# zhiqiangdon/pose-adv-aug

Measured on AMD Instinct MI355X. Metric: images/sec, 2-stack HG 256x256 bs=24 per GPU, full training step, higher is better.
Workload: dtype bf16; 1 GPU; BASELINE configs[1]: 2-stack hourglass chan 256, bs=24/GPU, 256x256 MPII-shape synthetic frames (720x1280 uint8 resident in HBM), on-device HumanAug warp, heat-map MSE, RMSprop, PCKh; global_batch=24, parallelism=dp1, ranks_seen=1, devices_seen=1

## Files before the change

### include/poseadv.h

```cpp
#ifndef POSEADV_H
#define POSEADV_H
#include <stddef.h>
#include <stdint.h>
#ifdef __cplusplus
extern "C" {
#endif

const char* pa_last_error(void);
int pa_version(void);
int pa_dtype(void);
float pa_grad_scale(void);


int pa_gaussian_heatmap(const double* pts, float* out, int B, int J, int H, int W, void* stream);

int pa_weighted_l2(const float* pred, const float* gt, const float* weight, size_t n, float* loss, void* stream);
int pa_weighted_l2_grad(const float* pred, const float* gt, const float* weight, size_t n, const float* gout_dev,
                        float* dpred, void* stream);

int pa_get_preds(const float* maps, int B, int J, int H, int W, float* preds, float* maxval, void* stream);

int pa_final_preds(const float* maps, const float* center, const float* scale, const float* rot,
                   int B, int J, int H, int W, float* out, float* scratch_preds, void* stream);

// ... 176 lines not shown
int pa_hg_set_image_grad(pa_net* net, float* dimg, int layout);

int pa_hg_forward_half(pa_net* net, const float* img, const void* img4, int train);

int pa_asn_forward(pa_net* asn, pa_net* pose, int train, float* logits_scale, float* logits_rot);
const float* pa_asn_probs(const pa_net* asn);
int pa_asn_backward(pa_net* asn, pa_net* pose, const float* target_scale, const float* target_rot, float* loss);
int pa_asn_set_log_eps(pa_net* asn, float eps);

int pa_asn_forward_masks(pa_net* asn, pa_net* pose, int train, float* mask_logits);
int pa_asn_backward_masks(pa_net* asn, pa_net* pose, const float* dlogits);
int pa_hg_set_dropout_masks(pa_net* net, const float* masks);

int pa_hg_accuracy(pa_net* net, int stack, const int32_t* idxs, int nidx, float* acc, float* scratch);

int pa_hg_pckh(pa_net* net, int stack, const float* center, const float* scale, const float* rot, const float* gt_pts,
               const float* norm, const int32_t* idxs, int nidx, float* acc, float* person, float* scratch);

int pa_net_meters_async(pa_net* net, int on);

#define PA_PROF_CLASSES 12
int pa_net_profile_begin(pa_net* net);
int pa_net_profile_report(pa_net* net, double* out_host, int cap_classes, int* n_classes);
int pa_net_profile_classes(const pa_net* net, int32_t* out_host, int cap);
int pa_net_set_fin_prologue(pa_net* net, int max_rows);
int pa_net_set_pool_route(pa_net* net, int on);
int pa_net_design_bytes(const pa_net* net, double* out_host);
int pa_copy_probe(void* dst, const void* src, size_t bytes, void* stream);
int pa_copy_probe_form(void* dst, const void* src, size_t bytes, int form, void* stream);
int pa_conv2d_time(int mode, int variant, int B, int Cin, int Cout, int H, int W, int k, int iters, void* ws, float* ms_out, void* stream);
int pa_conv_plan_describe(int B, int H, int W, int Cin, int Cout, int taps, int in_mode, int add1_mode, int add2_mode, int ep_mode,
                          int ep2_mode, int fin_rows, int flags, int cus, int* out, int cap);
int pa_conv_launch_log(int* out, int cap);

int pa_net_set_multi_stream(pa_net* net, int on);

int pa_hg_debug_tensor(pa_net* net, const char* which, int grad, float* out, int* shape4);

int pa_asn_debug_tensor(pa_net* net, const char* which, int grad, float* out, int* shape4);

#ifdef __cplusplus
}
#endif
#endif
```

### pose_adv_aug_amd/_lib.py

```python
import ctypes as C
import os

import torch

_HERE = os.path.dirname(os.path.abspath(__file__))
DTYPE = os.environ.get('POSEADV_DTYPE', 'bf16').lower()
if DTYPE not in ('bf16', 'fp16'):
    raise ValueError('POSEADV_DTYPE must be bf16 or fp16')
LIB_PATH = os.path.join(_HERE, 'libposeadv_hip.so' if DTYPE == 'bf16' else 'libposeadv_hip_fp16.so')


def set_dtype(name):
    global DTYPE, LIB_PATH
    name = name.lower()
    if name not in ('bf16', 'fp16'):
        raise ValueError('dtype must be bf16 or fp16')
    if _lib is not None and name != DTYPE:
        raise PoseAdvError('the %s library is already loaded in this process' % DTYPE)
    DTYPE = name
    LIB_PATH = os.path.join(_HERE, 'libposeadv_hip.so' if name == 'bf16' else 'libposeadv_hip_fp16.so')


def act_dtype():
    return torch.bfloat16 if DTYPE == 'bf16' else torch.float16
# ... 127 lines not shown
    'pa_hg_heatmap_nhwc': (_vp, [_vp, _i]),
    'pa_hg_heatmap_nchw': (_i, [_vp, _i, _vp]),
    'pa_hg_backward': (_i, [_vp]),
    'pa_hg_backward_phase': (_i, [_vp, _i]),
    'pa_hg_bucket_range': (_i, [_vp, _i, C.POINTER(_sz), C.POINTER(_sz)]),
    'pa_hg_bucket_wait': (_i, [_vp, _i, _vp]),
    'pa_hg_train_step': (_i, [_vp, _vp, _vp, _i, _i, _vp]),
    'pa_hg_set_loss_total': (_i, [_vp, _vp]),
    'pa_hg_set_heat_grads': (_i, [_vp, C.POINTER(_vp), _i]),
    'pa_hg_set_image_grad': (_i, [_vp, _vp, _i]),
    'pa_stem_dgrad_workspace_bytes': (_sz, [_i, _i, _i]),
    'pa_stem_dgrad': (_i, [_vp, _vp, _vp, _i, _i, _i, _i, _vp, _vp]),
    'pa_hg_accuracy': (_i, [_vp, _i, _vp, _i, _vp, _vp]),
    'pa_hg_forward_half': (_i, [_vp, _vp, _vp, _i]),
    'pa_asn_forward': (_i, [_vp, _vp, _i, _vp, _vp]),
    'pa_asn_probs': (_vp, [_vp]),
    'pa_asn_backward': (_i, [_vp, _vp, _vp, _vp, _vp]),
    'pa_asn_set_log_eps': (_i, [_vp, _f]),
    'pa_hg_pckh': (_i, [_vp, _i, _vp, _vp, _vp, _vp, _vp, _vp, _i, _vp, _vp, _vp]),
    'pa_net_meters_async': (_i, [_vp, _i]),
    'pa_net_profile_begin': (_i, [_vp]),
    'pa_net_profile_report': (_i, [_vp, C.POINTER(C.c_double), _i, C.POINTER(_i)]),
    'pa_net_design_bytes': (_i, [_vp, C.POINTER(C.c_double)]),
    'pa_copy_probe': (_i, [_vp, _vp, _sz, _vp]),
    'pa_copy_probe_form': (_i, [_vp, _vp, _sz, _i, _vp]),
    'pa_params_csr': (_i, [_vp, _i, _vp, _vp]),
    'pa_net_set_fin_prologue': (_i, [_vp, _i]),
    'pa_net_set_pool_route': (_i, [_vp, _i]),
    'pa_wgrad_group_workspace_bytes': (_sz, [_vp, _i]),
    'pa_wgrad_group': (_i, [_vp, _i, _i, _vp, _vp]),
    'pa_conv2d_time': (_i, [_i] * 9 + [_vp, C.POINTER(C.c_float), _vp]),
    'pa_conv_plan_describe': (_i, [_i] * 14 + [C.POINTER(_i), _i]),
    'pa_conv_launch_log': (_i, [C.POINTER(_i), _i]),
    'pa_net_profile_classes': (_i, [_vp, C.POINTER(C.c_int32), _i]),
    'pa_net_set_multi_stream': (_i, [_vp, _i]),
    'pa_hg_debug_tensor': (_i, [_vp, C.c_char_p, _i, _vp, C.POINTER(_i)]),
    'pa_asn_debug_tensor': (_i, [_vp, C.c_char_p, _i, _vp, C.POINTER(_i)]),
}

EXPORTS = sorted(_PROTOS)


def lib():
    global _lib
    if _lib is None:
        if not os.path.isfile(LIB_PATH):
            raise PoseAdvError('%s not found: run `python -c "import __graft_entry__ as g; g.build()"` '
                               '(there is no CPU fallback)' % LIB_PATH)
        try:
            l = C.CDLL(LIB_PATH)
        except OSError as e:
            raise PoseAdvError('cannot load %s: %s' % (LIB_PATH, e))
        for name, (res, args) in _PROTOS.items():
            fn = getattr(l, name)
            fn.restype = res
            fn.argtypes = args
        if l.pa_dtype() != (0 if DTYPE == 'bf16' else 1):
            raise PoseAdvError('%s is not the %s build' % (LIB_PATH, DTYPE))
        _lib = l
    return _lib


def check(rc, what=''):
    if rc != 0:
        msg = lib().pa_last_error()
        raise PoseAdvError('%s failed (code %d): %s' % (what or 'libposeadv_hip call', rc, msg.decode() if msg else ''))
# ... 26 lines not shown
```

### pose_adv_aug_amd/csrc/conv1x1_tile.hip

```cpp
#include "common.h"
#include "kernels.h"
#include "conv_epilogue.h"
#include <stdlib.h>

PA_STAMP_DECL(pa_conv1t_clk, pa_debug_conv1t_clocks)
#ifdef PA_TUNING
#define PA_STAMPT(i) do { if ((a.dbg & 64) && blockIdx.x == (unsigned)(a.dbg >> 8) && blockIdx.y == 0 && threadIdx.x == 0) { \
        pa_conv1t_clk[2 * (i)] = __builtin_amdgcn_s_memtime(); pa_conv1t_clk[2 * (i) + 1] = wall_clock64(); } } while (0)
#else
#define PA_STAMPT(i) do { } while (0)
#endif

#ifndef PA_CONV1_UP_OCC
#define PA_CONV1_UP_OCC(up) 3
#endif
#ifndef PA_CONV1_OCC4
#define PA_CONV1_OCC4(cin, bm, bn, ld) 4
#endif
#define PA_GLOBAL_PTR(p) ((const __attribute__((address_space(1))) void*)(p))
#define PA_LDS_PTR(p) ((__attribute__((address_space(3))) void*)(p))

constexpr bool pa_conv1_occ4_inst(int CIN, int BM, int BN, int LD, bool PIN) {
    if (CIN == 128 && BM == 64 && BN == 64) return LD == PA_LD_PLAIN || PIN;
    if (CIN == 64 && BM == 128 && BN == 64) return LD == PA_LD_BNRELU;
    if (CIN == 64 && BM == 64 && BN == 128) return LD == PA_LD_PLAIN || LD == PA_LD_LIN2;
    return false;
}
constexpr int pa_conv1_occ(int CIN, int BM, int BN, int LD, int KS, bool UP, bool PIN) {
    if (pa_conv1_occ4_inst(CIN, BM, BN, LD, PIN)) return PA_CONV1_OCC4(CIN, BM, BN, LD);
    if (((CIN == 128 || KS == 32) && BM == 64) || (CIN == 64 && (BN == 64 || BM == 64))) return PA_CONV1_UP_OCC(UP);
    return 2;
}
constexpr int pa_conv1_ks(int CIN, int BM, int BN, int LD) { return (CIN == 64 && BM == 64 && BN == 128 && pa_conv1_occ(CIN, BM, BN, LD, 64, false, false) == 4) ? 32 : 64; }

template <int CIN, int BM, int BN, int LDMODE, int KS = 64, bool UP = false, int POOL = PA_POOL_EP_NONE, bool PIN = false>
__global__ __launch_bounds__(256, pa_conv1_occ(CIN, BM, BN, LDMODE, KS, UP, PIN)) void conv1x1_tile_kernel(PaConvArgs a, int nb_per_wg) {
    constexpr bool OCC4 = pa_conv1_occ(CIN, BM, BN, LDMODE, KS, UP, PIN) == 4;
    constexpr int CPP = CIN / 8;
    constexpr int NI = BN / 32, MI = BM / 32;
    constexpr int KT = CIN / KS;
    constexpr int WRI = 512 / KS;
    constexpr int NIW = (BN / 4) / WRI;
    constexpr int PSTEP = 256 / CPP;
    constexpr int NPASS = BM / PSTEP;
    constexpr bool CTAB = (BM == 64 && ((CIN == 128 && LDMODE == PA_LD_LIN2) || KS == 32)) || (CIN == 64 && (BN == 64 || BM == 64));
    __shared__ __attribute__((aligned(16))) bf16 lds[BM * CIN + 2 * BN * KS + ((CTAB || OCC4) ? 2 * BN * 8 : 0)];
    bf16* As = lds;
    bf16* wbuf = lds + BM * CIN;

    const int tid = threadIdx.x, lane = tid & 63;
    const int wave = __builtin_amdgcn_readfirstlane(tid >> 6);
    const int wm = wave & 1, wn = wave >> 1;
    const int M = a.B * a.H * a.W;
    const int m0 = blockIdx.x * BM;
    const int nb0 = blockIdx.y * nb_per_wg;
    const int nit = nb_per_wg * KT;
    PA_SET_MAIN_PRIO();
    PA_STAMPT(0);
#ifdef PA_TUNING
    if ((a.dbg >> 16) > 0 && gridDim.x > 256) {
        const int slot = ((int)blockIdx.x / 256) % 3;
        for (int i = 0; i < slot * (a.dbg >> 16); ++i) __builtin_amdgcn_s_sleep(16);
    }
#endif
// ... 138 lines not shown
            asm volatile("s_waitcnt vmcnt(0)" ::: "memory");
            __syncthreads();
        }
        if (nbi == 0) PA_STAMPT(4);
        float* T = reinterpret_cast<float*>(KS == 32 ? wbuf : wbuf + ((nbi * KT + KT - 1) & 1) * (BN * KS));
        if constexpr (UP) {
            pa_conv_epilogue_lds_up<BN, NI, MI>(a, acc, (nb0 + nbi) * BN, wm, wn, pixel_of_row,
                                                [&](int x) { return up_rp * (a.W / 2) + up_cx * (BM / 4) + (x >> 1); },
                                                T, (int)blockIdx.x, reinterpret_cast<float4*>(lds + BM * CIN + 2 * BN * KS));
        } else
        pa_conv_epilogue_auto<BN, NI, MI, (CIN == 256 || CIN == 64 || CTAB), CTAB, 256, (BN < 128), POOL, OCC4>(a, acc, (nb0 + nbi) * BN, wm, wn,
                                         [&](int wr, int mi, int p) { const int m = m0 + wr * (BM / 2) + mi * 16 + p; return m < M ? m : -1; },
                                         T, (int)blockIdx.x, (CTAB || OCC4) ? reinterpret_cast<float4*>(lds + BM * CIN + 2 * BN * KS) : nullptr);
        if (nbi == 0) PA_STAMPT(5);
        __syncthreads();
    }
    PA_STAMPT(6);
}

template <int CIN, int BM, int BN, int KS = 64, bool LIN2_ONLY = false>
static void launch_row_ld(const PaConvArgs& a, int variant, dim3 grid, int nbw, hipStream_t st) {
    if constexpr (LIN2_ONLY) {
        hipLaunchKernelGGL((conv1x1_tile_kernel<CIN, BM, BN, PA_LD_LIN2, KS>), grid, dim3(256), 0, st, a, nbw);
    } else {
        switch (variant) {
            case PA_LD_PLAIN: hipLaunchKernelGGL((conv1x1_tile_kernel<CIN, BM, BN, PA_LD_PLAIN, KS>), grid, dim3(256), 0, st, a, nbw); break;
            case PA_LD_BNRELU: hipLaunchKernelGGL((conv1x1_tile_kernel<CIN, BM, BN, PA_LD_BNRELU, KS>), grid, dim3(256), 0, st, a, nbw); break;
            default: hipLaunchKernelGGL((conv1x1_tile_kernel<CIN, BM, BN, PA_LD_LIN2, KS>), grid, dim3(256), 0, st, a, nbw); break;
        }
    }
}

int pa_launch_conv1x1_tile(const PaConvArgs& a0, const PaConvPlan& p, hipStream_t st) {
    PaConvArgs a = a0; a.dbg = pa_tuning().conv1t_dbg;
    const dim3 grid(p.gx, p.gy); const int v = p.variant(), nbw = p.nbw;
    switch (p.tiling()) {
        case PA_CT_R128_64_128_UP: hipLaunchKernelGGL((conv1x1_tile_kernel<128, 64, 128, PA_LD_LIN2, 64, true>), grid, dim3(256), 0, st, a, nbw); break;
        case PA_CT_R128_64_64_PIN: hipLaunchKernelGGL((conv1x1_tile_kernel<128, 64, 64, PA_LD_LIN2, 64, false, PA_POOL_EP_NONE, true>), grid, dim3(256), 0, st, a, nbw); break;
        case PA_CT_R256_64_128_K32: launch_row_ld<256, 64, 128, 32>(a, v, grid, nbw, st); break;
        case PA_CT_R256_64_128: launch_row_ld<256, 64, 128>(a, v, grid, nbw, st); break;
        case PA_CT_R256_64_64: launch_row_ld<256, 64, 64>(a, v, grid, nbw, st); break;
        case PA_CT_R128_64_128:
            if (v == PA_CV_POOL_BWD) hipLaunchKernelGGL((conv1x1_tile_kernel<128, 64, 128, PA_LD_LIN2, 64, false, PA_POOL_EP_BWD>), grid, dim3(256), 0, st, a, nbw);
            else if (v == PA_CV_POOL_PLAIN) hipLaunchKernelGGL((conv1x1_tile_kernel<128, 64, 128, PA_LD_LIN2, 64, false, PA_POOL_EP_PLAIN>), grid, dim3(256), 0, st, a, nbw);
            else launch_row_ld<128, 64, 128>(a, v, grid, nbw, st);
            break;
        case PA_CT_R128_64_64: launch_row_ld<128, 64, 64>(a, v, grid, nbw, st); break;
        case PA_CT_R128_128_128: launch_row_ld<128, 128, 128, 64, true>(a, v, grid, nbw, st); break;
        case PA_CT_R128_128_64: launch_row_ld<128, 128, 64, 64, true>(a, v, grid, nbw, st); break;
        case PA_CT_R64_64_128:
            switch (v) {
                case PA_LD_PLAIN: hipLaunchKernelGGL((conv1x1_tile_kernel<64, 64, 128, PA_LD_PLAIN, pa_conv1_ks(64, 64, 128, PA_LD_PLAIN)>), grid, dim3(256), 0, st, a, nbw); break;
                case PA_LD_BNRELU: hipLaunchKernelGGL((conv1x1_tile_kernel<64, 64, 128, PA_LD_BNRELU, pa_conv1_ks(64, 64, 128, PA_LD_BNRELU)>), grid, dim3(256), 0, st, a, nbw); break;
                default: hipLaunchKernelGGL((conv1x1_tile_kernel<64, 64, 128, PA_LD_LIN2, pa_conv1_ks(64, 64, 128, PA_LD_LIN2)>), grid, dim3(256), 0, st, a, nbw); break;
            }
            break;
        case PA_CT_R64_128_128: launch_row_ld<64, 128, 128>(a, v, grid, nbw, st); break;
        case PA_CT_R64_128_64: launch_row_ld<64, 128, 64>(a, v, grid, nbw, st); break;
        default: pa_set_error_msg("pa_launch_conv1x1_tile: the plan names no instance of conv1x1_tile.hip"); return 1;
    }
    return (int)hipGetLastError();
}
```

### pose_adv_aug_amd/csrc/conv_epilogue.h

```cpp
#pragma once
#include "common.h"
#include "kernels.h"
#ifndef PA_EPI_LEAN_MG
#define PA_EPI_LEAN_MG 2
#endif
#ifndef PA_EPI_STAMP
#define PA_EPI_STAMP(i) do { } while (0)
#endif

template <int BN, int NI>
__device__ __forceinline__ int pa_weight_row_of_lds_row(int lr) {
    const int wt = lr / (BN / 2), l = lr - wt * (BN / 2);
    const int ni = l >> 4, rr = l & 15;
    return wt * (BN / 2) + 32 * (ni >> 1) + 8 * (rr >> 2) + 4 * (ni & 1) + (rr & 3);
}

template <int BN, int NI>
__device__ __forceinline__ int pa_lds_row_of_weight_row(int c) {
    const int wt = c / (BN / 2), l = c - wt * (BN / 2);
    const int ch = l >> 5, rem = l & 31;
    const int q = rem >> 3, h = (rem >> 2) & 1, j = rem & 3;
    return wt * (BN / 2) + (2 * ch + h) * 16 + 4 * q + j;
}

// ... 319 lines not shown
            } else {
                if constexpr (POOL) {
                    PaPoolRaw r;
                    pa_pool_request(a.add2, (unsigned)m, (unsigned)a.W, (unsigned)N, (unsigned)n, idx, r);
                    pa_read8(a.add1, idx, n, e1);
#pragma unroll
                    for (int j = 0; j < 8; ++j) e2[j] = pa_pool_value(r, pool_e, j);
                } else {
                pa_read8(a.add1, idx, n, e1);
                pa_read8(a.add2, idx, n, e2);
                }
            }
            bf16x8 o;
#pragma unroll
            for (int j = 0; j < 8; ++j) {
                float v = (j < 4 ? v0[j & 3] : v1[j & 3]) + bias[j] + e1[j] + e2[j];
                o[j] = (bf16)v;
                float rv = (float)o[j];
                s1[j] += rv;
                s2[j] += rv * rv;
            }
            *reinterpret_cast<bf16x8*>(a.out + idx) = o;
        }
        PA_EPI_STAMP(8 + 2 * mi);
    }
    if (a.ep.mode != PA_OUT_PLAIN) {
        PA_EPI_STAMP(11);
        pa_lds_barrier();
        const f32x2 v = pa_stats_reduce<BN, NT, TSMALL>(s1, s2, T);
        if (tid < BN) *reinterpret_cast<f32x2*>(a.ep.stats + ((size_t)stat_row * N + n0 + tid) * 2) = v;
    }
}

template <int BN, int NI, int MI, bool TAB, int NT = 256, bool TSMALL = false, bool FUSE = false, bool POOL = false, bool LEAN = false, class PixFn>
__device__ __forceinline__ void pa_conv_epilogue_lds_bwd(const PaConvArgs& a, f32x4 (&acc)[NI][MI], int n0, int wm, int wn,
                                                         PixFn pix, float* T, int stat_row, float4* ctab = nullptr) {
    constexpr int CPR = BN / 8;
    constexpr int RPS = NT / CPR;
    constexpr int SW = (NT / 8) / RPS;
    constexpr int NW = NT / 64;
    constexpr int G = FUSE ? MI : ((MI >= 2 && !TAB) ? 2 : 1);
    constexpr int ROWS = NT / 8;
    static_assert(!FUSE || !TAB, "fused staging: constants in registers");
    constexpr int IT = G * SW;
    int tid = threadIdx.x;
    if constexpr (LEAN) asm volatile("" : "+v"(tid));
    const int lane = tid & 63;
    const int N = a.Cout;
    const int chunk = tid % CPR, rsub = tid / CPR;
    const int n = n0 + chunk * 8;
    const int m1 = a.add1.mode, m2 = a.add2.mode;
    float s1[8], s2[8], es[8], et[8], ka[8], kb[8], kc[8];
#pragma unroll
    for (int j = 0; j < 8; ++j) { s1[j] = 0.f; s2[j] = 0.f; }
    const int wrow = wm * 16 + (lane & 15);
    const int wslot0 = (wn * (BN / 2)) / 4 + 2 * (lane >> 4);
#pragma unroll
    for (int g = 0; g < MI; g += G) {
        unsigned idx[IT];
        bool ok[IT];
        bf16x8 xr[IT], p1[IT], q1[IT], p2[POOL ? 1 : IT];
        PaPoolRaw pr[POOL ? IT : 1];
        const bool pool_e = POOL && a.add2.q != nullptr;
#pragma unroll
        for (int pp = 0; pp < G; ++pp)
#pragma unroll
            for (int sw = 0; sw < SW; ++sw) {
                const int it = pp * SW + sw, r = sw * RPS + rsub;
                const int m = pix(r >> 4, g + pp, r & 15);
                ok[it] = m >= 0;
                idx[it] = ok[it] ? (unsigned)m * (unsigned)N + (unsigned)n : 0u;
#ifdef PA_TUNING
                if (a.dbg & 16) { xr[it] = bf16x8{}; p1[it] = bf16x8{}; q1[it] = bf16x8{}; p2[it] = bf16x8{}; continue; }
#endif
// ... 119 lines not shown
                r0[j] = (float)o0[j]; r1[j] = (float)o1[j];
            }
            *reinterpret_cast<bf16x8*>(a.out + i0) = o0;
            *reinterpret_cast<bf16x8*>(a.out + i1) = o1;
        }
        bf16x8 ol;
#pragma unroll
        for (int j = 0; j < 8; ++j) {
            const float q0 = __shfl_xor(r0[j], 16, 64), q1 = __shfl_xor(r1[j], 16, 64);
            const float sum = ((r0[j] + q0) + r1[j]) + q1;
            const float4 e = ctab[j * CPR + chunk];
            const float xv = (float)xl[j];
            const float dz = (fmaf(e.x, xv, e.y) > 0.f) ? sum : 0.f;
            ol[j] = (bf16)dz;
            if (!(rsub & 1)) { const float dzr = (float)ol[j]; l1[j] += dzr; l2[j] += dzr * xv; }
        }
        if (!(rsub & 1)) *reinterpret_cast<bf16x8*>(a.out2 + il) = ol;
    }
    float cm = 0.f, ci = 0.f;
    if (tid < BN) { cm = a.ep2.mean[n0 + tid]; ci = a.ep2.invstd[n0 + tid]; }
    pa_lds_barrier();
    const f32x2 t = pa_stats_reduce<BN, NT, false>(l1, l2, T);
    if (tid < BN) {
        f32x2 v = {t[0], ci * (t[1] - cm * t[0])};
        *reinterpret_cast<f32x2*>(a.ep2.stats + ((size_t)stat_row * N + n0 + tid) * 2) = v;
    }
}

__host__ __device__ inline bool pa_bwd_epilogue_lds_ok(const PaConvArgs& a) {
    return a.xcd < 2 && a.bias == nullptr && (a.add1.mode == PA_LD_NONE || a.add1.mode == PA_LD_PLAIN || a.add1.mode == PA_LD_LIN2) &&
           (a.add2.mode == PA_LD_NONE || a.add2.mode == PA_LD_PLAIN);
}

template <int BN, int NI, int MI, bool BWD_LDS = true, bool TAB = false, int NT = 256, bool TSMALL = false, int POOL = 0, bool LEAN = false, class PixFn>
__device__ __forceinline__ void pa_conv_epilogue_auto(const PaConvArgs& a, f32x4 (&acc)[NI][MI], int n0, int wm, int wn,
                                                      PixFn pix, float* T, int stat_row, float4* ctab = nullptr) {
    constexpr bool FUSE = !TSMALL && !TAB && MI > 1 && MI * BN <= 128;
    if constexpr (POOL == PA_POOL_EP_BWD) {
        pa_conv_epilogue_lds_bwd<BN, NI, MI, TAB, NT, TSMALL, FUSE, true>(a, acc, n0, wm, wn, pix, T, stat_row, ctab);
        return;
    } else if constexpr (POOL == PA_POOL_EP_PLAIN) {
        pa_conv_epilogue_lds<BN, NI, MI, NT, TSMALL, FUSE, true>(a, acc, n0, wm, wn, pix, T, stat_row);
        return;
    }
    if (a.ep.mode == PA_OUT_BWD) {
        const bool lds_ok = BWD_LDS && pa_bwd_epilogue_lds_ok(a);
        if (lds_ok) {
            pa_conv_epilogue_lds_bwd<BN, NI, MI, (TAB || LEAN), NT, TSMALL, FUSE, false, LEAN>(a, acc, n0, wm, wn, pix, T, stat_row, ctab);
        } else if constexpr (TAB || NT != 256) {
            __builtin_trap();
        } else {
            const int p = threadIdx.x & 15;
            pa_conv_epilogue<BN, NI, MI, (LEAN && MI > PA_EPI_LEAN_MG) ? PA_EPI_LEAN_MG : MI>(a, acc, n0, wm, wn, [&](int mi) { return pix(wm, mi, p); }, T, stat_row);
        }
    } else {
        pa_conv_epilogue_lds<BN, NI, MI, NT, TSMALL, FUSE, false, LEAN>(a, acc, n0, wm, wn, pix, T, stat_row, ctab);
    }
}
```

### pose_adv_aug_amd/csrc/kernels.h

```cpp
#pragma once
#include "common.h"
#include "bn_fin.h"
#include "launch_plan.h"
#include "wgrad_plan.h"
#include "conv_plan.h"

struct PaConvArgs {
    PaOperand in;
    const bf16* w;
    const float* bias;
    PaOperand add1;
    PaOperand add2;
    PaEpilogue ep;
    bf16* out;
    int B, H, W, Cin, Cout, taps;
    bf16* dz_out;
    PaBnFin fin;
    int low_prio;
    int dbg;
    int xcd;
    PaEpilogue ep2;
    bf16* out2;
};
int pa_conv_cus();
inline PaConvShape pa_conv_shape(const PaConvArgs& a) {
    return PaConvShape{a.B, a.H, a.W, a.Cin, a.Cout, a.taps, a.in.mode, a.add1.mode, a.add2.mode, a.ep.mode, a.ep2.mode, a.fin.rows, a.bias != nullptr,
                       a.out2 != nullptr, a.dz_out != nullptr, a.in.map != nullptr, a.in.q != nullptr, a.ep2.scale && a.ep2.shift, a.add2.map != nullptr,
                       pa_conv_cus()};
}
int pa_launch_conv(const PaConvArgs& a, const PaConvPlan& p, hipStream_t st, int* stat_rows = nullptr);
inline int pa_launch_conv(const PaConvArgs& a, hipStream_t st, int* stat_rows = nullptr) { return pa_launch_conv(a, pa_conv_plan(pa_conv_shape(a)), st, stat_rows); }
int pa_launch_conv3x3_tile(const PaConvArgs& a, const PaConvPlan& p, hipStream_t st);
int pa_launch_conv1x1_tile(const PaConvArgs& a, const PaConvPlan& p, hipStream_t st);
inline int pa_max_stat_rows(int M) { int r = (M + 63) / 64; return r < 512 ? 512 : r; }

struct PaWgradArgs {
    PaOperand dy;
    PaOperand x;
    float* part;
    float* dbpart;
    int B, H, W, Cin, Cout, taps, splits;
};
int pa_launch_wgrad(const PaWgradArgs& a, hipStream_t st);
int pa_launch_stem_wgrad_tile(const PaWgradArgs& a, const PaWgradPlan& p, hipStream_t st);
int pa_launch_wgrad_tile(const PaWgradArgs& a, const PaWgradPlan& p, hipStream_t st);
int pa_wgrad_job_workgroups(const PaWgradArgs& a);
struct PaWgradReduceJob;
int pa_launch_wgrad_group(const PaWgradArgs* const* jobs, int n, hipStream_t st, bool keep_order = false,
                          const PaWgradReduceJob* red_jobs = nullptr, const int* red_idx = nullptr, int red_n = 0);
void pa_wgrad_set_launch_flags(unsigned flags);

struct PaWgradReduceJob {
    const float* part; float* dst; const float* dbpart; float* dbdst;
    int Cout, Cin, taps, splits, real_cout, real_cin;
};
int pa_launch_wgrad_reduce(const PaWgradReduceJob* jobs_dev, int njobs, int max_elems, hipStream_t st);
#define PA_RED_LIST_MAX 24
struct PaRedList { int idx[PA_RED_LIST_MAX]; };
int pa_launch_wgrad_reduce_list(const PaWgradReduceJob* jobs_dev, const int* idx, int n, int max_elems, hipStream_t st);

int pa_launch_bn_fin(const PaBnFin& f, int C, hipStream_t st);
int pa_launch_bn_fin2(const PaBnFin& a, int Ca, const PaBnFin& b, int Cb, hipStream_t st);
struct PaBnEvalJob { const float* gamma; const float* beta; const float* rmean; const float* rvar; float* scale; float* shift; int C; };
int pa_launch_bn_eval(const PaBnEvalJob* jobs_dev, int njobs, float eps, hipStream_t st);

int pa_launch_maxpool_fwd(const PaOperand& in, bf16* out, int B, int H, int W, int C, hipStream_t st, unsigned char* map = nullptr, bf16* xmax = nullptr);
// ... 63 lines not shown
```

### pose_adv_aug_amd/csrc/tuning.h

```cpp
#pragma once
#include <stdlib.h>

#define PA_TUNING_TABLE(X)                                                                                                           \
                                                                      \
    X(conv1_old,        "PA_CONV1_OLD",        0,   "1x1 convolutions on the generic kernel (no row-tile kernel, no fused upsample-add gradient)") \
    X(conv3_old,        "PA_CONV3_OLD",        0,   "3x3 convolutions on the generic kernel (no halo-tile kernel)")                 \
    X(wgrad_old,        "PA_WGRAD_OLD",        0,   "weight gradients on the generic kernel (no tile kernel, stem included)")       \
    X(stem_wgrad_old,   "PA_STEM_WGRAD_OLD",   0,   "the stem's weight gradient on the generic kernel")                            \
    X(eltwise_old,      "PA_ELTWISE_OLD",      0,   "pooling / upsample-add / cell-mask launches in their first, unvectorised form") \
    X(conv3_nosmall,    "PA_CONV3_NOSMALL",    0,   "no 8 x 8 / 4 x 4 halo tiles: the small maps go to the generic kernel")        \
    X(igemm_oneshot,    "PA_IGEMM_ONESHOT",    1,   "0: the small 1x1 layers on the K-stepping generic kernel instead of the one-shot one") \
    X(no_dz3,           "PA_NO_DZ3",           0,   "conv3's data gradient does not store dz3 (its readers recompute it)")         \
    X(no_dz2,           "PA_NO_DZ2",           0,   "conv2's data gradient does not store dz2")                                    \
    X(epi_bwd_direct,   "PA_EPI_BWD_DIRECT",   0,   "direct (no LDS) BatchNorm-backward epilogue wherever an instance carries both") \
    X(conv3_noxcd,      "PA_CONV3_NOXCD",      0,   "3x3 tiles in launch order instead of one contiguous range per XCD")           \
    X(wg_group,         "PA_WG_GROUP",         1,   "0: one launch per weight gradient instead of group launches")                 \
    X(wg_red_in_group,  "PA_WG_RED_IN_GROUP",  1,   "0: slab reductions as launches of their own instead of inside the next group launch") \
    X(wgrad_anyorder,   "PA_WGRAD_ANYORDER",   1,   "0: ungrouped weight gradients of one flush as ordinary in-order launches")    \
    X(wgrad_nopipe,     "PA_WGRAD_NOPIPE",     0,   "plain instead of pipelined tile weight gradients")                            \
    X(upadd_fuse,       "PA_UPADD_FUSE",       1,   "0: the upsample-add backward's low-resolution half as a launch of its own")   \
    X(upadd_split,      "PA_UPADD_SPLIT",      1,   "0: both halves of the upsample-add backward in one launch on the main stream") \
    X(pool_route,       "PA_POOL_ROUTE",       3,   "pool gradients through the forward pools' arg-max maps: bit 0 the hourglass pools, bit 1 the stem's pool (0: a pool backward launch each)") \
    X(fin_prologue,     "PA_FIN_PROLOGUE",     128, "most partial rows a consumer finalizes in its prologue (0: always a finalize launch; at most 128)") \
    X(fin_mask,         "PA_FIN_MASK",         7,   "which finalizes may ride in a consumer: 1 forward x1 / x2, 2 backward x2, 4 backward x3") \
    X(single_stream,    "PA_SINGLE_STREAM",    0,   "everything on the caller's stream")                                           \
    X(no_wstream,       "PA_NO_WSTREAM",       0,   "side streams, but the weight gradients on the stream that produced their operands") \
    X(stem_on_main,     "PA_STEM_ON_MAIN",     1,   "0: the stem's weight gradient on the weight-gradient stream")                 \
                                                              \
    X(wgrad_wgs1,       "PA_WGRAD_WGS1",       256, "workgroup target of a 1x1 tile weight gradient launched alone")               \
    X(wgrad_wgs9,       "PA_WGRAD_WGS9",       256, "the same for 3x3")                                                            \
    X(wgrad_min1,       "PA_WGRAD_MIN1",       3,   "fewest 128-pixel tiles for which a 1x1 weight gradient takes the tile kernel") \
    X(wg_group_wgs1,    "PA_WG_GROUP_WGS1",    64,  "workgroup budget of a 1x1 job of a group launch")                             \
    X(wg_group_wgs9,    "PA_WG_GROUP_WGS9",    64,  "the same for 3x3")                                                            \
    X(wg_group_minper1, "PA_WG_GROUP_MINPER1", 2,   "fewest tiles per workgroup of a 1x1 job")                                     \
    X(wg_group_minper9, "PA_WG_GROUP_MINPER9", 4,   "the same for 3x3")                                                            \
    X(wg_group_cap,     "PA_WG_GROUP_CAP",     256, "most workgroups of one group launch")                                         \
    X(wg_red_wgs,       "PA_WG_RED_WGS",       256, "workgroups of the slab reduction inside a group launch")                      \
    X(wreduce_lag,      "PA_WREDUCE_LAG",      2,   "flushes whose slabs wait in the stash before they are summed")                \
    X(stem_splits,      "PA_STEM_SPLITS",      512, "splits (slabs) of the stem's weight gradient")                                \
    X(wgrad_tile1,      "PA_WGRAD_TILE1",      0,   "generic 1x1 weight gradient: forced tile variant (0: by shape)")              \
    X(wgrad_tile9,      "PA_WGRAD_TILE9",      0,   "the same for 3x3")                                                            \
    X(wgrad_blocks,     "PA_WGRAD_BLOCKS",     0,   "generic weight gradient: forced split count (0: by shape)")                   \
                                                                                    \
    X(ablate,           "PA_ABLATE",           0,   "INSTRUMENT, wrong results: mask of launch classes that are skipped (net.hip)") \
    X(ablate_h,         "PA_ABLATE_H",         8,   "INSTRUMENT: largest map height the low-resolution bits of PA_ABLATE skip")    \
    X(conv3_dbg,        "PA_CONV3_DBG",        0,   "INSTRUMENT, wrong results: phase ablation / tap rotation / cycle stamps of the 3x3 tile kernel") \
    X(conv1_dbg,        "PA_CONV1_DBG",        0,   "INSTRUMENT, timing only: cycle stamps of the one-shot 1x1 kernel")            \
    X(conv1t_dbg,       "PA_CONV1T_DBG",       0,   "INSTRUMENT, timing only: cycle stamps of the row-tile 1x1 kernel")            \
    X(fin_anyorder,     "PA_FIN_ANYORDER",     0,   "INSTRUMENT, results may be wrong: finalize launches without ordering behind their producer")

struct PaTuning {
#define PA_TUNING_FIELD(field, env, value, doc) int field = value;
    PA_TUNING_TABLE(PA_TUNING_FIELD)
#undef PA_TUNING_FIELD
};

#ifdef PA_TUNING
inline const PaTuning& pa_tuning() {
    static const PaTuning t = [] {
        PaTuning v;
#define PA_TUNING_READ(field, env, value, doc) if (const char* e = getenv(env)) v.field = atoi(e);
        PA_TUNING_TABLE(PA_TUNING_READ)
#undef PA_TUNING_READ
        return v;
    }();
    return t;
}
#else
inline const PaTuning& pa_tuning() {
    static constexpr PaTuning t{};
    return t;
}
// ... 2 lines not shown
```

Baseline: 4296 images/sec.

## Add persistent multi-tile 1x1 conv kernel that keeps weights resident in LDS

Result: no change. 4313 images/sec (median of 4 runs) (+0.4%).

```diff
diff --git a/include/poseadv.h b/include/poseadv.h
--- a/include/poseadv.h
+++ b/include/poseadv.h
@@ -232,6 +232,8 @@
 int pa_conv_plan_describe(int B, int H, int W, int Cin, int Cout, int taps, int in_mode, int add1_mode, int add2_mode, int ep_mode,
                           int ep2_mode, int fin_rows, int flags, int cus, int* out, int cap);
 int pa_conv_launch_log(int* out, int cap);
+int pa_conv1_stream_set(int mode);
+int pa_conv1_stream_launches(long long* out, int cap);
 
 int pa_net_set_multi_stream(pa_net* net, int on);
 
diff --git a/pose_adv_aug_amd/_lib.py b/pose_adv_aug_amd/_lib.py
--- a/pose_adv_aug_amd/_lib.py
+++ b/pose_adv_aug_amd/_lib.py
@@ -183,6 +183,8 @@
     'pa_conv2d_time': (_i, [_i] * 9 + [_vp, C.POINTER(C.c_float), _vp]),
     'pa_conv_plan_describe': (_i, [_i] * 14 + [C.POINTER(_i), _i]),
     'pa_conv_launch_log': (_i, [C.POINTER(_i), _i]),
+    'pa_conv1_stream_set': (_i, [_i]),
+    'pa_conv1_stream_launches': (_i, [C.POINTER(C.c_longlong), _i]),
     'pa_net_profile_classes': (_i, [_vp, C.POINTER(C.c_int32), _i]),
     'pa_net_set_multi_stream': (_i, [_vp, _i]),
     'pa_hg_debug_tensor': (_i, [_vp, C.c_char_p, _i, _vp, C.POINTER(_i)]),
diff --git a/pose_adv_aug_amd/csrc/conv1x1_stream.hip b/pose_adv_aug_amd/csrc/conv1x1_stream.hip
--- /dev/null
+++ b/pose_adv_aug_amd/csrc/conv1x1_stream.hip
@@ -0,0 +1,243 @@
+#include "common.h"
+#include "kernels.h"
+#include "conv_epilogue.h"
+#include "tuning.h"
+#include <atomic>
+
+#define PA_GLOBAL_PTR(p) ((const __attribute__((address_space(1))) void*)(p))
+#define PA_LDS_PTR(p) ((__attribute__((address_space(3))) void*)(p))
+
+#ifndef PA_STREAM_EPG
+#define PA_STREAM_EPG(mi) 2
+#endif
+constexpr bool stream_ep_tab(int CIN, int BM, int LD) { return CIN == 64 || (BM == 64 && CIN == 128 && LD == PA_LD_LIN2); }
+
+template <int CIN, int BM, int LDMODE, bool PIN = false>
+__global__ __launch_bounds__(256, 3) void conv1x1_stream_kernel(PaConvArgs a, int tpw, int ntiles) {
+    constexpr int BN = 64;
+    constexpr int CPP = CIN / 8;
+    constexpr int NI = BN / 32, MI = BM / 32;
+    constexpr int KT = CIN / 64;
+    constexpr int PSTEP = 256 / CPP, NPASS = BM / PSTEP;
+    constexpr bool TAB = stream_ep_tab(CIN, BM, LDMODE), LEAN = true;
+    constexpr int NK = LDMODE == PA_LD_PLAIN ? 0 : LDMODE == PA_LD_BNRELU ? 2 : PIN ? 5 : 3;
+    static_assert(BM * CIN * 2 >= 32 * BN * 4 && BM * CIN * 2 >= 256 * 8 * 4 && NPASS * PSTEP == BM, "the dead activation tile is the epilogue tile");
+    __shared__ __attribute__((aligned(16))) bf16 lds[BN * CIN + BM * CIN + 2 * BN * 8 + (NK ? NK : 1) * CIN * 2];
+    bf16* wres = lds;
+    bf16* As = lds + BN * CIN;
+    float* T = reinterpret_cast<float*>(As);
+    float4* ctab = reinterpret_cast<float4*>(As + BM * CIN);
+    float* ktab = reinterpret_cast<float*>(As + BM * CIN + 2 * BN * 8);
+
+    const int tid = threadIdx.x, lane = tid & 63;
+    const int wave = __builtin_amdgcn_readfirstlane(tid >> 6);
+    const int wm = wave & 1, wn = wave >> 1;
+    const int M = a.B * a.H * a.W;
+    const int chunk = tid % CPP, c = chunk * 8, prow = tid / CPP;
+    PA_SET_MAIN_PRIO();
+
+    float kv[NK ? NK : 1];
+    if constexpr (NK > 0) {
+        static_assert(CIN <= 256, "one table entry per thread and row");
+#pragma unroll
+        for (int r = 0; r < NK; ++r) {
+            const float* src = r == 0 ? a.in.k0 : r == 1 ? a.in.k1 : r == 2 ? a.in.k2 : r == 3 ? a.ep2.scale : a.ep2.shift;
+            kv[r] = src[tid < CIN ? tid : 0];
+        }
+    }
+#pragma unroll
+    for (int kh = 0; kh < KT; ++kh)
+#pragma unroll
+        for (int i = 0; i < 2; ++i) {
+            const int lr = wave * 16 + i * 8 + (lane >> 3);
+            const int wr = pa_weight_row_of_lds_row<BN, NI>(lr);
+            const int wc = ((lane & 7) ^ (lr & 7)) << 3;
+            __builtin_amdgcn_global_load_lds(PA_GLOBAL_PTR(a.w + (size_t)wr * CIN + kh * 64 + wc),
+                                             PA_LDS_PTR(wres + kh * (BN * 64) + (wave * 16 + i * 8) * 64), 16, 0, 0);
+        }
+
+    bf16x8 ra[NPASS], rq[LDMODE == PA_LD_LIN2 ? NPASS : 1];
+    uint2 rmp[PIN ? NPASS : 1];
+    unsigned rpos[PIN ? NPASS : 1];
+    auto request = [&](int tile) {
+        const int m0 = min(tile, ntiles - 1) * BM;
+#pragma unroll
+        for (int u = 0; u < NPASS; ++u) {
+            const int m = m0 + u * PSTEP + prow;
+            const size_t idx = m < M ? (size_t)m * CIN + c : 0;
+            if constexpr (PIN) {
+                const unsigned mm = m < M ? (unsigned)m : 0u, rowg = mm / (unsigned)a.W, x = mm - rowg * (unsigned)a.W;
+                const size_t lo = (size_t)((rowg >> 1) * ((unsigned)a.W >> 1) + (x >> 1)) * CIN + c;
+                rpos[u] = ((rowg & 1u) << 1) | (x & 1u);
+                ra[u] = *reinterpret_cast<const bf16x8*>(a.in.p + lo);
+                rmp[u] = *reinterpret_cast<const uint2*>(a.in.map + lo);
+            } else
+            ra[u] = *reinterpret_cast<const bf16x8*>(a.in.p + idx);
+            if constexpr (LDMODE == PA_LD_LIN2) rq[u] = *reinterpret_cast<const bf16x8*>(a.in.q + idx);
+        }
+    };
+    auto stage = [&](int tile) {
+        const int m0 = tile * BM;
+        float k0[8], k1[8], k2[8], ps[8], pt[8];
+        if constexpr (NK > 0) {
+#pragma unroll
+            for (int h = 0; h < 2; ++h) {
+                const f32x4 v0 = *reinterpret_cast<const f32x4*>(ktab + c + 4 * h), v1 = *reinterpret_cast<const f32x4*>(ktab + CIN + c + 4 * h);
+#pragma unroll
+                for (int j = 0; j < 4; ++j) { k0[4 * h + j] = v0[j]; k1[4 * h + j] = v1[j]; }
+                if constexpr (LDMODE == PA_LD_LIN2) {
+                    const f32x4 v2 = *reinterpret_cast<const f32x4*>(ktab + 2 * CIN + c + 4 * h);
+#pragma unroll
+                    for (int j = 0; j < 4; ++j) k2[4 * h + j] = v2[j];
+                }
+                if constexpr (PIN) {
+                    const f32x4 v3 = *reinterpret_cast<const f32x4*>(ktab + 3 * CIN + c + 4 * h), v4 = *reinterpret_cast<const f32x4*>(ktab + 4 * CIN + c + 4 * h);
+#pragma unroll
+                    for (int j = 0; j < 4; ++j) { ps[4 * h + j] = v3[j]; pt[4 * h + j] = v4[j]; }
+                }
+            }
+        }
+#pragma unroll
+        for (int u = 0; u < NPASS; ++u) {
+            const int row = u * PSTEP + prow, m = m0 + row;
+            bf16x8 o;
+            if constexpr (LDMODE == PA_LD_PLAIN) {
+                o = ra[u];
+            } else if constexpr (LDMODE == PA_LD_BNRELU) {
+#pragma unroll
+                for (int j = 0; j < 8; ++j) o[j] = (bf16)fmaxf(fmaf(k0[j], (float)ra[u][j], k1[j]), 0.f);
+            } else if constexpr (PIN) {
+#pragma unroll
+                for (int j = 0; j < 8; ++j) {
+                    const unsigned b = ((j < 4 ? rmp[u].x : rmp[u].y) >> (8 * (j & 3))) & 0xffu;
+                    const float q = (float)rq[u][j];
+                    const float r = (b == rpos[u] ? (float)ra[u][j] : 0.f) + 0.f;
+                    const float dz = (float)(bf16)((fmaf(ps[j], q, pt[j]) > 0.f) ? r : 0.f);
+                    o[j] = (bf16)fmaf(k0[j], dz, fmaf(k1[j], q, k2[j]));
+                }
+            } else {
+#pragma unroll
+                for (int j = 0; j < 8; ++j)
+                    o[j] = (bf16)fmaf(k0[j], (float)ra[u][j], fmaf(k1[j], (float)rq[u][j], k2[j]));
+            }
+            if (m >= M) {
+#pragma unroll
+                for (int j = 0; j < 8; ++j) o[j] = (bf16)0.f;
+            }
+            const int sw = CPP >= 16 ? (row & 15) : ((row >> 1) & 7);
+            *reinterpret_cast<bf16x8*>(As + row * CIN + ((chunk ^ sw) << 3)) = o;
+            if (LDMODE == PA_LD_LIN2 && a.dz_out && m < M)
+                *reinterpret_cast<bf16x8*>(a.dz_out + (size_t)m * CIN + c) = o;
+        }
+    };
+
+    const int t0 = (int)blockIdx.x * tpw;
+    request(t0);
+    if constexpr (NK > 0) {
+#pragma unroll
+        for (int r = 0; r < NK; ++r)
+            if (tid < CIN) ktab[r * CIN + tid] = kv[r];
+    }
+    pa_lds_barrier();
+
+    const int frow = lane & 15, fchk = lane >> 4;
+    for (int s = 0; s < tpw; ++s) {
+        const int tile = t0 + s;
+        if (tile >= ntiles) break;
+        stage(tile);
+        if (s == 0) asm volatile("s_waitcnt vmcnt(0)" ::: "memory");
+        pa_lds_barrier();
+        request(tile + 1);
+        f32x4 acc[NI][MI];
+#pragma unroll
+        for (int ni = 0; ni < NI; ++ni)
+#pragma unroll
+            for (int mi = 0; mi < MI; ++mi) acc[ni][mi] = f32x4{0.f, 0.f, 0.f, 0.f};
+#pragma unroll
+        for (int kh = 0; kh < KT; ++kh) {
+            const bf16* Bs = wres + kh * (BN * 64);
+#pragma unroll
+            for (int kk = 0; kk < 2; ++kk) {
+                bf16x8 fa[MI], fw[NI];
+                const int ch = kh * 8 + kk * 4 + fchk;
+#pragma unroll
+                for (int mi = 0; mi < MI; ++mi) {
+                    const int row = wm * (BM / 2) + mi * 16 + frow;
+                    const int sw = CPP >= 16 ? (row & 15) : ((row >> 1) & 7);
+                    fa[mi] = *reinterpret_cast<const bf16x8*>(As + row * CIN + ((ch ^ sw) << 3));
+                }
+#pragma unroll
+                for (int ni = 0; ni < NI; ++ni) {
+                    const int row = wn * (BN / 2) + ni * 16 + frow;
+                    fw[ni] = *reinterpret_cast<const bf16x8*>(Bs + row * 64 + (((fchk + 4 * kk) ^ (row & 7)) << 3));
+                }
+#pragma unroll
+                for (int ni = 0; ni < NI; ++ni)
+#pragma unroll
+                    for (int mi = 0; mi < MI; ++mi)
+                        acc[ni][mi] = PA_MFMA_16x16x32(fw[ni], fa[mi], acc[ni][mi]);
+            }
+        }
+        pa_lds_barrier();
+        const int m0 = tile * BM;
+        pa_conv_epilogue_auto<BN, NI, MI, (CIN == 64 || TAB), TAB, 256, true, PA_POOL_EP_NONE, LEAN, PA_STREAM_EPG(MI)>(a, acc, 0, wm, wn,
+                                         [&](int wr, int mi, int p) { const int m = m0 + wr * (BM / 2) + mi * 16 + p; return m < M ? m : -1; },
+                                         T, tile, ctab);
+        pa_lds_barrier();
+    }
+}
+
+enum { ST_64_PLAIN, ST_64_BNRELU, ST_64_LIN2, ST_128_PLAIN, ST_128_LIN2, ST_128_PIN, ST_COUNT };
+static std::atomic<int> g_mode{-1};
+static std::atomic<long long> g_taken[ST_COUNT];
+static bool stream_paid(int i) { return (pa_tuning().conv1_stream_inst >> i) & 1; }
+static int stream_tpw(int i) { const int t = pa_tuning().conv1_stream_tpw; return t > 0 ? t : i < ST_128_PLAIN ? 2 : 4; }
+
+int pa_conv1_stream_mode() { const int m = g_mode.load(std::memory_order_relaxed); return m < 0 ? pa_tuning().conv1_stream : m; }
+
+static int stream_instance(const PaConvArgs& a, const PaConvPlan& p) {
+    if (p.gy != 1 || p.nbw != 1 || p.rows != p.gx || a.Cout != 64 || a.out2 || a.fin.rows > 0) return -1;
+    if (a.add2.mode == PA_LD_POOL) return -1;
+    switch (p.tiling()) {
+        case PA_CT_R64_128_64:
+            return p.variant() == PA_LD_PLAIN ? ST_64_PLAIN : p.variant() == PA_LD_BNRELU ? ST_64_BNRELU : p.variant() == PA_LD_LIN2 ? ST_64_LIN2 : -1;
+        case PA_CT_R128_64_64: return p.variant() == PA_LD_PLAIN ? ST_128_PLAIN : p.variant() == PA_LD_LIN2 ? ST_128_LIN2 : -1;
+        case PA_CT_R128_64_64_PIN: return ST_128_PIN;
+        default: return -1;
+    }
+}
+
+int pa_conv1_stream_tpw(const PaConvArgs& a, const PaConvPlan& p, bool force) {
+    const int i = stream_instance(a, p);
+    return i < 0 || !(force || stream_paid(i)) ? 0 : stream_tpw(i);
+}
+
+int pa_launch_conv1x1_stream(const PaConvArgs& a, const PaConvPlan& p, hipStream_t st) {
+    const int i = stream_instance(a, p);
+    if (i < 0) { pa_set_error_msg("pa_launch_conv1x1_stream: no instance of conv1x1_stream.hip carries this launch"); return 1; }
+    const int ntiles = p.gx, tpw = stream_tpw(i);
+    const dim3 grid((ntiles + tpw - 1) / tpw);
+    switch (i) {
+        case ST_64_PLAIN: hipLaunchKernelGGL((conv1x1_stream_kernel<64, 128, PA_LD_PLAIN>), grid, dim3(256), 0, st, a, tpw, ntiles); break;
+        case ST_64_BNRELU: hipLaunchKernelGGL((conv1x1_stream_kernel<64, 128, PA_LD_BNRELU>), grid, dim3(256), 0, st, a, tpw, ntiles); break;
+        case ST_64_LIN2: hipLaunchKernelGGL((conv1x1_stream_kernel<64, 128, PA_LD_LIN2>), grid, dim3(256), 0, st, a, tpw, ntiles); break;
+        case ST_128_PLAIN: hipLaunchKernelGGL((conv1x1_stream_kernel<128, 64, PA_LD_PLAIN>), grid, dim3(256), 0, st, a, tpw, ntiles); break;
+        case ST_128_LIN2: hipLaunchKernelGGL((conv1x1_stream_kernel<128, 64, PA_LD_LIN2>), grid, dim3(256), 0, st, a, tpw, ntiles); break;
+        default: hipLaunchKernelGGL((conv1x1_stream_kernel<128, 64, PA_LD_LIN2, true>), grid, dim3(256), 0, st, a, tpw, ntiles); break;
+    }
+    g_taken[i].fetch_add(1, std::memory_order_relaxed);
+    return (int)hipGetLastError();
+}
+
+extern "C" int pa_conv1_stream_set(int mode) {
+    if (mode < 0 || mode > 2) { pa_set_error_msg("pa_conv1_stream_set: mode is 0 (off), 1 (on) or 2 (force)"); return -1; }
+    for (auto& t : g_taken) t.store(0, std::memory_order_relaxed);
+    const int prev = pa_conv1_stream_mode();
+    g_mode.store(mode, std::memory_order_relaxed);
+    return prev;
+}
+extern "C" int pa_conv1_stream_launches(long long* out, int cap) {
+    if (!out || cap < ST_COUNT) { pa_set_error_msg("pa_conv1_stream_launches: out is NULL or holds fewer than 6 counts"); return -1; }
+    for (int i = 0; i < ST_COUNT; ++i) out[i] = g_taken[i].load(std::memory_order_relaxed);
+    return ST_COUNT;
+}
diff --git a/pose_adv_aug_amd/csrc/conv1x1_tile.hip b/pose_adv_aug_amd/csrc/conv1x1_tile.hip
--- a/pose_adv_aug_amd/csrc/conv1x1_tile.hip
+++ b/pose_adv_aug_amd/csrc/conv1x1_tile.hip
@@ -30,6 +30,13 @@
     if (pa_conv1_occ4_inst(CIN, BM, BN, LD, PIN)) return PA_CONV1_OCC4(CIN, BM, BN, LD);
     if (((CIN == 128 || KS == 32) && BM == 64) || (CIN == 64 && (BN == 64 || BM == 64))) return PA_CONV1_UP_OCC(UP);
     return 2;
+}
+static bool pa_conv1_stream_takes(const PaConvArgs& a, const PaConvPlan& p) {
+    const int mode = pa_conv1_stream_mode();
+    if (mode == 0) return false;
+    const int tpw = pa_conv1_stream_tpw(a, p, mode == 2);
+    if (tpw == 0) return false;
+    return mode == 2 || (pa_conv_cus() > 0 && p.gx >= 2 * tpw * 3 * pa_conv_cus());
 }
 constexpr int pa_conv1_ks(int CIN, int BM, int BN, int LD) { return (CIN == 64 && BM == 64 && BN == 128 && pa_conv1_occ(CIN, BM, BN, LD, 64, false, false) == 4) ? 32 : 64; }
 
@@ -234,6 +241,7 @@
 }
 
 int pa_launch_conv1x1_tile(const PaConvArgs& a0, const PaConvPlan& p, hipStream_t st) {
+    if (pa_conv1_stream_takes(a0, p)) return pa_launch_conv1x1_stream(a0, p, st);
     PaConvArgs a = a0; a.dbg = pa_tuning().conv1t_dbg;
     const dim3 grid(p.gx, p.gy); const int v = p.variant(), nbw = p.nbw;
     switch (p.tiling()) {
diff --git a/pose_adv_aug_amd/csrc/conv_epilogue.h b/pose_adv_aug_amd/csrc/conv_epilogue.h
--- a/pose_adv_aug_amd/csrc/conv_epilogue.h
+++ b/pose_adv_aug_amd/csrc/conv_epilogue.h
@@ -375,14 +375,15 @@
     }
 }
 
-template <int BN, int NI, int MI, bool TAB, int NT = 256, bool TSMALL = false, bool FUSE = false, bool POOL = false, bool LEAN = false, class PixFn>
+template <int BN, int NI, int MI, bool TAB, int NT = 256, bool TSMALL = false, bool FUSE = false, bool POOL = false, bool LEAN = false, int GO = 0, class PixFn>
 __device__ __forceinline__ void pa_conv_epilogue_lds_bwd(const PaConvArgs& a, f32x4 (&acc)[NI][MI], int n0, int wm, int wn,
                                                          PixFn pix, float* T, int stat_row, float4* ctab = nullptr) {
     constexpr int CPR = BN / 8;
     constexpr int RPS = NT / CPR;
     constexpr int SW = (NT / 8) / RPS;
     constexpr int NW = NT / 64;
-    constexpr int G = FUSE ? MI : ((MI >= 2 && !TAB) ? 2 : 1);
+    constexpr int G = GO ? GO : FUSE ? MI : ((MI >= 2 && !TAB) ? 2 : 1);
+    static_assert(MI % G == 0, "whole groups of passes");
     constexpr int ROWS = NT / 8;
     static_assert(!FUSE || !TAB, "fused staging: constants in registers");
     constexpr int IT = G * SW;
@@ -568,7 +569,7 @@
            (a.add2.mode == PA_LD_NONE || a.add2.mode == PA_LD_PLAIN);
 }
 
-template <int BN, int NI, int MI, bool BWD_LDS = true, bool TAB = false, int NT = 256, bool TSMALL = false, int POOL = 0, bool LEAN = false, class PixFn>
+template <int BN, int NI, int MI, bool BWD_LDS = true, bool TAB = false, int NT = 256, bool TSMALL = false, int POOL = 0, bool LEAN = false, int BWD_G = 0, class PixFn>
 __device__ __forceinline__ void pa_conv_epilogue_auto(const PaConvArgs& a, f32x4 (&acc)[NI][MI], int n0, int wm, int wn,
                                                       PixFn pix, float* T, int stat_row, float4* ctab = nullptr) {
     constexpr bool FUSE = !TSMALL && !TAB && MI > 1 && MI * BN <= 128;
@@ -582,7 +583,7 @@
     if (a.ep.mode == PA_OUT_BWD) {
         const bool lds_ok = BWD_LDS && pa_bwd_epilogue_lds_ok(a);
         if (lds_ok) {
-            pa_conv_epilogue_lds_bwd<BN, NI, MI, (TAB || LEAN), NT, TSMALL, FUSE, false, LEAN>(a, acc, n0, wm, wn, pix, T, stat_row, ctab);
+            pa_conv_epilogue_lds_bwd<BN, NI, MI, (TAB || LEAN), NT, TSMALL, FUSE, false, LEAN, BWD_G>(a, acc, n0, wm, wn, pix, T, stat_row, ctab);
         } else if constexpr (TAB || NT != 256) {
             __builtin_trap();
         } else {
diff --git a/pose_adv_aug_amd/csrc/kernels.h b/pose_adv_aug_amd/csrc/kernels.h
--- a/pose_adv_aug_amd/csrc/kernels.h
+++ b/pose_adv_aug_amd/csrc/kernels.h
@@ -32,6 +32,9 @@
 inline int pa_launch_conv(const PaConvArgs& a, hipStream_t st, int* stat_rows = nullptr) { return pa_launch_conv(a, pa_conv_plan(pa_conv_shape(a)), st, stat_rows); }
 int pa_launch_conv3x3_tile(const PaConvArgs& a, const PaConvPlan& p, hipStream_t st);
 int pa_launch_conv1x1_tile(const PaConvArgs& a, const PaConvPlan& p, hipStream_t st);
+int pa_conv1_stream_mode();
+int pa_conv1_stream_tpw(const PaConvArgs& a, const PaConvPlan& p, bool force);
+int pa_launch_conv1x1_stream(const PaConvArgs& a, const PaConvPlan& p, hipStream_t st);
 inline int pa_max_stat_rows(int M) { int r = (M + 63) / 64; return r < 512 ? 512 : r; }
 
 struct PaWgradArgs {
diff --git a/pose_adv_aug_amd/csrc/tuning.h b/pose_adv_aug_amd/csrc/tuning.h
--- a/pose_adv_aug_amd/csrc/tuning.h
+++ b/pose_adv_aug_amd/csrc/tuning.h
@@ -38,6 +38,9 @@
     X(wg_red_wgs,       "PA_WG_RED_WGS",       256, "workgroups of the slab reduction inside a group launch")                      \
     X(wreduce_lag,      "PA_WREDUCE_LAG",      2,   "flushes whose slabs wait in the stash before they are summed")                \
     X(stem_splits,      "PA_STEM_SPLITS",      512, "splits (slabs) of the stem's weight gradient")                                \
+    X(conv1_stream,     "PA_CONV1_STREAM",     1,   "the multi-tile 1x1 kernel until pa_conv1_stream_set is called: 0 off, 1 on, 2 every launch an instance carries") \
+    X(conv1_stream_inst, "PA_CONV1_STREAM_INST", 4,  "instances of conv1x1_stream.hip that pa_conv1_stream_set(1) takes: bit 0 - 2 64 -> 64 plain / BatchNorm + ReLU / BatchNorm backward, bit 3 - 5 128 -> 64 plain / BatchNorm backward / pool-routed") \
+    X(conv1_stream_tpw, "PA_CONV1_STREAM_TPW", 0,   "row tiles per workgroup of the multi-tile 1x1 kernel (0: 2 for 128-row tiles, 4 for 64-row tiles)") \
     X(wgrad_tile1,      "PA_WGRAD_TILE1",      0,   "generic 1x1 weight gradient: forced tile variant (0: by shape)")              \
     X(wgrad_tile9,      "PA_WGRAD_TILE9",      0,   "the same for 3x3")                                                            \
     X(wgrad_blocks,     "PA_WGRAD_BLOCKS",     0,   "generic weight gradient: forced split count (0: by shape)")                   \
```
